# swift-nav/albatross

Measured on AMD Instinct MI355X. Metric: GP fits/sec (Gram+Chol+solve) at N=16384 fp64, higher is better.
Workload: dtype f64

## Files before the change

albatross_amd/csrc/api.hip:

```cpp
#include <algorithm>
#include <atomic>
#include <cmath>
#include <cstring>
#include <chrono>
#include <cstdio>
#include <new>
#include <thread>

#include "api_internal.h"
#include <deque>
#include <mutex>
#include <tuple>
#include <unordered_map>
#include "trace.h"
#include "pub.h"

namespace agp {

void DeviceFeatures::release() {
  for (void *&p : owned) {
    if (p) (void)hipFree(p);
    p = nullptr;
  }
  v = FeatView{};
// ... 146 lines not shown
  auto number = [](const char *name, long long dflt) {
    const char *e = getenv(name);
    return e && e[0] ? atoll(e) : dflt;
  };
  t.panel_fused = flag("AGP_PANEL_FUSED", true);
  t.step_below = number("AGP_STEP_BELOW", 4608);
  t.gram_sop = flag("AGP_GRAM_SOP", true);
  t.backsub_coop = flag("AGP_BACKSUB_COOP", true);
  t.backsub_coop_max = number("AGP_BACKSUB_COOP_MAX", BACKSUB_COOP_MAX_N);
  t.mixed_bf16 = flag("AGP_MIXED_BF16", true);
  t.mixed_f16 = flag("AGP_MIXED_F16", true);
  set_f16x2_kernel((int)number("AGP_F16X2_LDS_PAD", 8192), (int)number("AGP_F16X2_TERMS", 4), (int)number("AGP_F16X2_CHUNK", 32));
  t.mixed_nbo = number("AGP_MIXED_NBO", 512);
  t.fp64_nbo = number("AGP_FP64_NBO", 0);
  if (t.fp64_nbo <= 512 || t.fp64_nbo % 128 != 0) t.fp64_nbo = 0;
  set_bf16x3_kernel((int)number("AGP_BF16X3_KERNEL", 2), (int)number("AGP_BF16X3_LDS_PAD", 8192));
  t.sparse_pivoted = flag("AGP_SPARSE_PIVOTED", false);
  t.predict_chunk = number("AGP_PREDICT_CHUNK", 0);
  t.shard_block = number("AGP_SHARD_BLOCK", 0);
  t.shard_force_comm = flag("AGP_SHARD_FORCE_COMM", false);
  t.shard_host_pacing = flag("AGP_SHARD_HOST_PACING", false);
  if (const char *e = getenv("AGP_SHARD_MASK_GFLOP")) t.shard_mask_gflop = atof(e);
  t.merge_above = number("AGP_MERGE_ABOVE", 8704);
  return t;
}

int agp_context_create(int device_id, agp_context **out) {
  if (!out) return AGP_ERR_INVALID_ARGUMENT;
  *out = nullptr;
  int n = 0;
  if (hipGetDeviceCount(&n) != hipSuccess || n <= 0) return AGP_ERR_NO_DEVICE;
  if (device_id < 0 || device_id >= n) return AGP_ERR_INVALID_ARGUMENT;
  agp_context_impl *ctx = new (std::nothrow) agp_context_impl();
  if (!ctx) return AGP_ERR_INVALID_ARGUMENT;
  ctx->device = device_id;
  ctx->tune = read_tuning();
  agp::g_gram_sop = ctx->tune.gram_sop;
  AGP_HIP_CHECK(ctx, hipSetDevice(device_id));
  {
    int lo = 0, hi = 0;
    AGP_HIP_CHECK(ctx, hipDeviceGetStreamPriorityRange(&lo, &hi));
    AGP_HIP_CHECK(ctx, hipStreamCreateWithPriority(&ctx->stream, hipStreamNonBlocking, hi));
    AGP_HIP_CHECK(ctx, hipStreamCreateWithPriority(&ctx->stream2, hipStreamNonBlocking, lo));
    AGP_HIP_CHECK(ctx, hipStreamCreateWithPriority(&ctx->stream3, hipStreamNonBlocking, lo));
    AGP_HIP_CHECK(ctx, hipEventCreateWithFlags(&ctx->ev_inv, hipEventDisableTiming));
    AGP_HIP_CHECK(ctx, hipEventCreateWithFlags(&ctx->ev_c, hipEventDisableTiming));
// ... 33 lines not shown
  ctx->helpers.clear();
  for (auto &sl : ctx->ext.slots)
    if (sl.dev) (void)hipFree(sl.dev);
  for (auto e : ctx->gemm_events) (void)hipEventDestroy(e);
  for (auto e : ctx->stage_ev)
    if (e) (void)hipEventDestroy(e);
  if (ctx->partial_ws) (void)hipFree(ctx->partial_ws);
  if (ctx->ws_A) (void)agp::dev_release(ctx->ws_A);
  if (ctx->pool_A) (void)agp::dev_release(ctx->pool_A);
  if (ctx->pool_K) (void)agp::dev_release(ctx->pool_K);
  if (ctx->ws_refine) (void)hipFree(ctx->ws_refine);
  if (ctx->p32) (void)hipFree(ctx->p32);
  if (ctx->f16_scales) (void)hipFree(ctx->f16_scales);
  if (ctx->pool_L32) (void)hipFree(ctx->pool_L32);
  if (ctx->pool_aux) (void)agp::dev_release(ctx->pool_aux);
  if (ctx->pool_shard) (void)agp::dev_release(ctx->pool_shard);
  if (ctx->pool_sparse) (void)agp::dev_release(ctx->pool_sparse);
  if (ctx->pool_batch) (void)agp::dev_release(ctx->pool_batch);
  if (ctx->ws_aux) (void)hipFree(ctx->ws_aux);
  if (ctx->d_zpub) (void)hipFree(ctx->d_zpub);
  if (ctx->d_dpub) (void)hipFree(ctx->d_dpub);
  if (ctx->shard_flags) (void)hipFree(ctx->shard_flags);
  if (ctx->d_headcnt) (void)hipFree(ctx->d_headcnt);
  if (ctx->h_stage) (void)hipHostFree(ctx->h_stage);
  if (ctx->d_flags) (void)hipFree(ctx->d_flags);
  if (ctx->h_flags) (void)hipHostFree(ctx->h_flags);
  if (ctx->ev_a) (void)hipEventDestroy(ctx->ev_a);
  if (ctx->ev_b) (void)hipEventDestroy(ctx->ev_b);
  if (ctx->stream) (void)hipStreamDestroy(ctx->stream);
  if (ctx->stream2) (void)hipStreamDestroy(ctx->stream2);
  if (ctx->stream3) (void)hipStreamDestroy(ctx->stream3);
  if (ctx->ev_inv) (void)hipEventDestroy(ctx->ev_inv);
  if (ctx->stream_masked) (void)hipStreamDestroy(ctx->stream_masked);
  if (ctx->stream_comm) (void)hipStreamDestroy(ctx->stream_comm);
  if (ctx->ev_c) (void)hipEventDestroy(ctx->ev_c);
  delete ctx;
  agp::dev_cache_trim();
}

int agp_context_synchronize(agp_context *ctx) {
  if (!ctx) return AGP_ERR_INVALID_ARGUMENT;
  AGP_HIP_CHECK(ctx, hipSetDevice(ctx->device));
  AGP_HIP_CHECK(ctx, hipDeviceSynchronize());
  return AGP_OK;
}

// ... 1652 lines not shown
```

albatross_amd/csrc/chol.hip:

```cpp
#include <cstdlib>
#include "common.h"
#include "mfma_f64.h"
#include "gemm_tiles.h"
#include "trsm_kernel.h"
#include "pub.h"

namespace agp {
void launch_set_identity_batched(hipStream_t s, double *B, long long ld, long long stride, long long m, long long count);

__device__ __forceinline__ double readlane_f64(double v, int lane) {
  const long long b = __double_as_longlong(v);
  const int lo = __builtin_amdgcn_readlane((int)(b & 0xffffffffll), lane);
  const int hi = __builtin_amdgcn_readlane((int)(b >> 32), lane);
  return __longlong_as_double(((long long)hi << 32) | (unsigned int)lo);
}

__device__ __forceinline__ double rsqrt_nr(double x) {
  double y = __builtin_amdgcn_rsq(x);
  const double h = 0.5 * x;
  y = y * (1.5 - h * y * y);
  y = y * (1.5 - h * y * y);
  return y;
}

struct PotrfArgs {
  double *A;
  long long lda;
  long long k0;
  int nbk;
  double *img;
  double *y;
// ... 803 lines not shown
  const long long cnt_img = (b1 - b0) * (long long)IMG_DOUBLES, cnt_z = k_end - k_begin;
  if (ctx->d_dpub && ctx->dpub_cap >= b1) {
    prep->fill(ctx->d_rowcnt + 2 * b0, 0ull, 2 * (b1 - b0));
    prep->sentinel(ctx->d_dpub + b0 * (long long)IMG_DOUBLES, cnt_img);
  }
  prep->sentinel(invd + b0 * (long long)IMG_DOUBLES, cnt_img);
  prep->sentinel(ctx->d_zpub + k_begin, cnt_z);
  if (want_step && k_begin == 0 && ctx->d_headcnt && ctx->tune.merge_above > 0 && k_end > ctx->tune.merge_above && !prep->full()) {
    prep->fill(ctx->d_headcnt, 0ull, agp_context::HEADCNT_WORDS);
    ctx->headcnt_ready = true;
  }
  ctx->zpub_ready_n = k_end;
  ctx->img_ready = invd;
  return true;
}

void panel_fused_prepare(agp_context *ctx, hipStream_t s, double *invd, long long k_begin, long long k_end, bool want_step) {
  PrepArgs prep;
  if (panel_fused_plan(ctx, invd, k_begin, k_end, want_step, &prep)) launch_prep(s, prep);
}

static void panel_phase(agp_context *ctx, hipStream_t s, double *A, long long n, long long lda, double *invd,
                        double *y, long long K0, long long kend, FactorTimers *timers, bool step_mode = false,
                        long long mark_after = -1, hipEvent_t mark_event = nullptr) {
  if (kend != n) step_mode = false;
  const bool inner_left = !step_mode && (n - K0) > INNER_LEFT_ABOVE;
  const bool fused = ctx->tune.panel_fused && ctx->d_zpub && ctx->zpub_ready_n >= kend && ctx->img_ready == invd &&
                     ((n - K0) <= FUSED_BELOW || step_mode);
  for (long long k = K0; k < kend; k += NB) {
    const int nbk = (int)((n - k < NB) ? n - k : NB);
    if (mark_event && k == mark_after + NB) (void)hipEventRecord(mark_event, s);
    if (inner_left && k > K0) {
      const double *P = A + K0 * lda + k;
      timed_gemm(s, timers, A + k * lda + k, lda, P, P, n - k, nbk, k - K0, false);
    }
    const long long below = n - (k + nbk);
    if (fused) {
      PotrfArgs pa;
      pa.A = A; pa.lda = lda; pa.k0 = k; pa.nbk = nbk;
      pa.img = invd + (k / NB) * (long long)IMG_DOUBLES;
      pa.y = y ? y + k : nullptr;
      pa.flags = ctx->d_flags; pa.scalars = ctx->d_scalars;
      pa.zpub = y ? ctx->d_zpub + k : nullptr;
      pa.below = below > 0 ? below : 0;
      if (step_mode && k > K0) {
        pa.dpub = ctx->d_dpub + (k / NB) * (long long)IMG_DOUBLES;
        unsigned grid = (unsigned)(1 + UPD_BLOCKS + (pa.below + 63) / 64);
        if (pa.below > 0) {
          const long long nt = (pa.below + 63) / 64;
          pa.trail_first = grid;
// ... 32 lines not shown
      ++ctx->sched.panels_split;
      if (below <= 0) continue;
      TrsmArgs t;
      t.img = invd + (k / NB) * (long long)IMG_DOUBLES;
      t.nbk = nbk;
      t.Y = A + k * lda + (k + nbk);
      t.stride_m = lda; t.stride_n = 1;
      t.ncols = below;
      t.z = y ? y + k : nullptr;
      t.yrest = y ? y + k + nbk : nullptr;
      t.batch_img = t.batch_Y = 0; t.n_total = 0;
      const unsigned grid = (unsigned)((below + 63) / 64);
      if (y) hipLaunchKernelGGL((trsm_micro_kernel<false, true>), dim3(grid), dim3(256), 0, s, t);
      else hipLaunchKernelGGL((trsm_micro_kernel<false, false>), dim3(grid), dim3(256), 0, s, t);
    }
    const long long width = kend - (k + nbk);
    if (width > 0 && !inner_left && !(step_mode && fused)) {
      const double *P = A + k * lda + (k + nbk);
      timed_gemm(s, timers, A + (k + nbk) * lda + (k + nbk), lda, P, P, below, width, nbk, false);
    }
  }
}

__global__ __launch_bounds__(64) void head_gate_kernel(const unsigned long long *done, unsigned long long expect, int *flags) {
  if (threadIdx.x == 0) {
    const unsigned long long t0 = __builtin_amdgcn_s_memrealtime();
    for (int spin = 1; __hip_atomic_load(done, __ATOMIC_RELAXED, __HIP_MEMORY_SCOPE_AGENT) < expect; ++spin) {
      if ((spin & 63) == 0 && poll_expired(t0, flags)) break;
      __builtin_amdgcn_s_sleep(16);
    }
    __atomic_thread_fence(__ATOMIC_ACQUIRE);
  }
}

void launch_head_gate(hipStream_t s, const unsigned long long *done, unsigned long long expect, int *flags) {
  hipLaunchKernelGGL(head_gate_kernel, dim3(1), dim3(64), 0, s, done, expect, flags);
}

static bool host_wait_event(hipEvent_t ev) {
  for (;;) {
    const hipError_t e = hipEventQuery(ev);
    if (e == hipSuccess) return true;
    if (e != hipErrorNotReady) { (void)hipGetLastError(); return false; }
    for (int i = 0; i < 32; ++i) __builtin_ia32_pause();
  }
}
// ... 48 lines not shown
  hipStream_t sa = ctx->stream, sb = ctx->stream2;
  hipStream_t sb_prev = sb;
  bool have_u2 = false, p32_flip = false;
  agp_context::ScheduleRecord &rec = ctx->sched;
  rec.reset_factor(n);
  long long K0 = 0, step_index = 0;
  const long long nbo_fixed = ctx->nbo_override;
  int variant = ctx->update_variant;
  const double *rs16 = nullptr, *irs16 = nullptr;
  if (variant == 5) {
    if (ctx->f16_scales && ctx->f16_scales_n >= n) {
      launch_f16x2_row_scales(sa, A, lda, n, ctx->f16_scales, ctx->f16_scales + ctx->f16_scales_n);
      rs16 = ctx->f16_scales;
      irs16 = ctx->f16_scales + ctx->f16_scales_n;
    } else {
      variant = 4;
    }
  }
  const long long nbo_wide = (variant == 4 || variant == 5) ? ctx->nbo_wide : ctx->tune.fp64_nbo;
  long long kend = K0 + pick_nbo(n, nbo_fixed, nbo_wide);
  if (kend > n) kend = n;
  if (!(ctx->prep_external && ctx->img_ready == invd && ctx->zpub_ready_n >= n)) panel_fused_prepare(ctx, sa, invd, 0, n, true);
  ctx->prep_external = false;
  auto step_ok = [&](long long remaining) { return nbo_fixed == 0 && step_fits(ctx, remaining) && step_ready(ctx, invd, n); };
  const bool step_all = step_ok(n);
  if (step_all) kend = n;
  const bool early_inv = step_all && ctx->bs_W && ctx->bs_done == 0 && ctx->ev_inv && ctx->stream2 && ctx->bs_BW > 0 &&
                         n % ctx->bs_BW == 0 && n / ctx->bs_BW >= 2;
  rec.add_step(kend, step_all ? rec.STEP : 0u);
  panel_phase(ctx, sa, A, n, lda, invd, y, K0, kend, timers, step_all, early_inv ? (n / ctx->bs_BW - 1) * ctx->bs_BW - NB : -1,
              early_inv ? ctx->ev_c : nullptr);
  if (early_inv) {
    const long long BW = ctx->bs_BW, done = n / BW - 1;
    if (host_wait_event(ctx->ev_c)) {
      hipStream_t si = ctx->stream2;
      launch_set_identity_batched(si, ctx->bs_W, BW, BW * BW, BW, done);
      forward_solve_mat_batched(si, A, BW * (lda + 1), BW, lda, invd, (BW / NB) * (long long)IMG_DOUBLES, ctx->bs_W, BW * BW, BW, BW,
                                true, done);
      (void)hipEventRecord(ctx->ev_inv, si);
      ctx->bs_done = done;
      rec.inv_bits |= rec.INV_EARLY;
    }
  }
  while (kend < n) {
    long long next_end = kend + pick_nbo(n - kend, nbo_fixed, nbo_wide);
    if (next_end > n) next_end = n;
    const long long K = kend - K0;
    const bool step = step_ok(n - kend);
    const bool single = !step && nbo_fixed == 0 && n - kend <= SINGLE_BELOW;
    if (step || single) next_end = n;
    if (ctx->bs_W && ctx->bs_done == 0 && next_end == n && ctx->ev_inv && ctx->stream2) {
      const long long BW = ctx->bs_BW, done = kend / BW;
      if (done > 0) {
        hipStream_t si = ctx->stream2;
        (void)hipEventRecord(ctx->ev_c, sa);
        (void)hipStreamWaitEvent(si, ctx->ev_c, 0);
        if (have_u2) (void)hipStreamWaitEvent(si, ctx->ev_b, 0);
        launch_set_identity_batched(si, ctx->bs_W, BW, BW * BW, BW, done);
        forward_solve_mat_batched(si, A, BW * (lda + 1), BW, lda, invd, (BW / NB) * (long long)IMG_DOUBLES, ctx->bs_W, BW * BW, BW, BW,
                                  true, done);
        (void)hipEventRecord(ctx->ev_inv, si);
        ctx->bs_done = done;
        rec.inv_bits |= rec.INV_LAST_STEP;
      }
    }
    const double *P = A + K0 * lda + kend;
    const float *P32 = nullptr;
    long long ld32 = 0;
    const unsigned short *P16 = nullptr;
    if (variant == 3 && ctx->p32 && (n - kend) >= U1_F32_ABOVE) {
      ld32 = (n - kend + 7) / 8 * 8;
      if (ld32 % 512 == 0) ld32 += 8;
      if (sizeof(float) * (size_t)ld32 * (size_t)K * 2 <= ctx->p32_bytes) {
        float *dst = ctx->p32 + (size_t)(p32_flip ? 1 : 0) * (ctx->p32_bytes / sizeof(float) / 2);
        p32_flip = !p32_flip;
        launch_convert_panel_f32(sa, P, lda, n - kend, K, dst, ld32);
        P32 = dst;
      }
    } else if (variant == 4 && ctx->p32 && (n - kend) >= U1_F32_ABOVE && K % 32 == 0 && 2 * bf16x3_bytes(n - kend, K) <= ctx->p32_bytes) {
      unsigned short *dst = reinterpret_cast<unsigned short *>(ctx->p32) + (size_t)(p32_flip ? 1 : 0) * (ctx->p32_bytes / sizeof(unsigned short) / 2);
      p32_flip = !p32_flip;
      launch_convert_panel_bf16x3(sa, P, lda, n - kend, K, dst);
      P16 = dst;
// ... 6 lines not shown
    (void)hipEventRecord(ctx->ev_a, sa);
    const bool merged = variant <= 0 && nbo_fixed == 0 && !step && next_end < n && ctx->headcnt_ready && ctx->tune.merge_above > 0 &&
                        (n - kend) > ctx->tune.merge_above && step_index < agp_context::HEADCNT_WORDS && (next_end - kend) % NB == 0;
    if (merged) {
      sb = (ctx->stream_masked && (n - kend) <= MASK_BELOW) ? ctx->stream_masked : ctx->stream2;
      if (sb != sb_prev && have_u2) (void)hipStreamWaitEvent(sb, ctx->ev_b, 0);
      sb_prev = sb;
      (void)hipStreamWaitEvent(sb, ctx->ev_a, 0);
      BulkTiming bt;
      const bool timed = timers && timers->ev && timers->used + 2 <= timers->n_ev;
      if (timed) { bt.e0 = timers->ev[timers->used]; bt.e1 = timers->ev[timers->used + 1]; }
      long long head_tiles = 0;
      unsigned long long *cnt = ctx->d_headcnt + step_index;
      launch_trailing_update_merged(sb, A + kend * lda + kend, lda, P, lda, n - kend, K, (int)((next_end - kend) / NB), cnt, &head_tiles,
                                    timed ? &bt : nullptr);
      if (timed && bt.flops > 0.) {
        timers->flops[timers->used / 2] = bt.flops;
        timers->used += 2;
      }
      (void)hipEventRecord(ctx->ev_b, sb);
      have_u2 = true;
      launch_head_gate(sa, cnt, (unsigned long long)head_tiles, ctx->d_flags);
      rec.add_step(next_end, rec.MERGED | (sb == ctx->stream_masked ? rec.MASKED : 0u));
      panel_phase(ctx, sa, A, n, lda, invd, y, kend, next_end, timers, false);
      K0 = kend;
      kend = next_end;
      ++step_index;
      continue;
    }
    ++step_index;
    if (have_u2) (void)hipStreamWaitEvent(sa, ctx->ev_b, 0);
    if (P16 && variant == 5) {
      launch_update_f16x2(sa, A + kend * lda + kend, lda, P16, n - kend, 0, 0, irs16 + kend, n - kend, next_end - kend, K);
    } else if (P16) {
      launch_update_bf16x3(sa, A + kend * lda + kend, lda, P16, n - kend, 0, 0, n - kend, next_end - kend, K);
    } else if ((variant == 3 || variant == 4 || variant == 5) && (n - kend) >= U1_F32_ABOVE) {
      launch_update_f32(sa, A + kend * lda + kend, lda, P, P, lda, n - kend, next_end - kend, K, P32, P32, ld32);
    } else if (step && n - kend > 1536) {
      timed_gemm(sa, timers, A + kend * lda + kend, lda, P, P, n - kend, n - kend, K, true, variant >= 4 ? 3 : variant);
    } else {
      timed_gemm(sa, timers, A + kend * lda + kend, lda, P, P, n - kend, next_end - kend, K, false);
    }
    sb = (ctx->stream_masked && (n - kend) <= MASK_BELOW) ? ctx->stream_masked : ctx->stream2;
    if (sb != sb_prev && have_u2) (void)hipStreamWaitEvent(sb, ctx->ev_b, 0);
    sb_prev = sb;
    const bool throttle = next_end < n && (n - kend) <= THROTTLE_BELOW;
    rec.add_step(next_end, (step ? rec.STEP : 0u) | (throttle ? rec.THROTTLED : 0u) | (single ? rec.SINGLE : 0u) |
                               (next_end < n && sb == ctx->stream_masked ? rec.MASKED : 0u));
    if (throttle) panel_phase(ctx, sa, A, n, lda, invd, y, kend, next_end, timers, step);
    if (next_end < n) {
      if (throttle) {
        if (!host_wait_event(ctx->ev_a)) (void)hipStreamWaitEvent(sb, ctx->ev_a, 0);
      } else {
        (void)hipStreamWaitEvent(sb, ctx->ev_a, 0);
      }
      const double *Q = A + K0 * lda + next_end;
      if (P16) {
        const long long M2 = n - next_end;
        const int ntr = (int)((M2 + 127) / 128);
        const long long tiles = (long long)ntr * (ntr + 1) / 2;
        long long olen = 0;
        const int *order = tiles >= 1024 ? bulk_tile_order(ntr, tiles, &olen) : nullptr;
        if (variant == 5)
          launch_update_f16x2(sb, A + next_end * lda + next_end, lda, P16, n - kend, next_end - kend, next_end - kend, irs16 + kend, M2, M2, K,
                              order, olen);
        else
          launch_update_bf16x3(sb, A + next_end * lda + next_end, lda, P16, n - kend, next_end - kend, next_end - kend, M2, M2, K, order, olen);
      } else
      timed_gemm(sb, timers, A + next_end * lda + next_end, lda, Q, Q, n - next_end, n - next_end, K, true, variant >= 4 ? 3 : variant,
                 P32 ? P32 + (next_end - kend) : nullptr, ld32);
      (void)hipEventRecord(ctx->ev_b, sb);
      have_u2 = true;
    } else {
      have_u2 = false;
    }
    const long long bw = ctx->bs_BW;
    const bool tail_inv = !throttle && step && next_end == n && ctx->bs_W && bw > 0 && ctx->ev_inv && ctx->stream2 && n % bw == 0 &&
                          ctx->bs_done > 0 && ctx->bs_done == kend / bw && n / bw - 1 > ctx->bs_done && (n / bw - 1) * bw - NB >= kend;
    if (!throttle) panel_phase(ctx, sa, A, n, lda, invd, y, kend, next_end, timers, step, tail_inv ? (n / bw - 1) * bw - NB : -1,
                               tail_inv ? ctx->ev_c : nullptr);
    if (tail_inv) {
      const long long first = ctx->bs_done, last = n / bw - 1, cnt = last - first;
      if (host_wait_event(ctx->ev_c)) {
        hipStream_t si = ctx->stream2;
        launch_set_identity_batched(si, ctx->bs_W + first * bw * bw, bw, bw * bw, bw, cnt);
        forward_solve_mat_batched(si, A + first * bw * (lda + 1), bw * (lda + 1), bw, lda, invd + first * (bw / NB) * (long long)IMG_DOUBLES,
                                  (bw / NB) * (long long)IMG_DOUBLES, ctx->bs_W + first * bw * bw, bw * bw, bw, bw, true, cnt);
        (void)hipEventRecord(ctx->ev_inv, si);
        ctx->bs_done = last;
        rec.inv_bits |= rec.INV_TAIL;
      }
    }
    K0 = kend;
    kend = next_end;
  }
  ctx->img_ready = nullptr;
  ctx->headcnt_ready = false;
}

bool batched_fused_fits(agp_context *ctx, long long n, long long count) {
  if (!ctx->tune.panel_fused || n <= NB) return false;
  const long long per_problem = 1 + (n - NB + 63) / 64;
  return count * per_problem <= step_slots(ctx);
}

void factor_lower_batched(hipStream_t s, double *A, long long stride_A, long long n, long long lda, double *invd,
                          long long stride_invd, double *y, long long stride_y, long long count, int *flags,
                          double *logsum, long long stride_flags, double *zpub, long long stride_zpub) {
  if (count <= 0 || n <= 0) return;
  const bool fused = zpub != nullptr && y != nullptr;
  for (long long K0 = 0; K0 < n; K0 += NBO) {
    const long long kend = (K0 + NBO < n) ? K0 + NBO : n;
    for (long long k = K0; k < kend; k += NB) {
      const int nbk = (int)((n - k < NB) ? n - k : NB);
      if (k > K0) {
        const double *P = A + K0 * lda + k;
        launch_gemm_nt_sub_batched(s, A + k * lda + k, lda, stride_A, P, lda, false, stride_A, P, lda, false, stride_A, n - k, nbk,
// ... 102 lines not shown
```

albatross_amd/csrc/common.h:

```cpp
#pragma once
#include <hip/hip_runtime.h>
#include <cstdint>
#include <cstdio>
#include <string>
#include <utility>
#include <vector>

#include "../../include/albatross_amd.h"
#include "cov_eval.h"

#define AGP_CHAIN_PRIO 3

namespace agp {

constexpr int NB = 128;
constexpr int NBO = 512;
constexpr int MB = 16;
constexpr int NMB = NB / MB;

struct FeatView {
  const double *coords;
  const long long *ids;
  const double *scales;
  long long n;
// ... 68 lines not shown
  double *d_zpub = nullptr;
  long long zpub_cap = 0, zpub_ready_n = 0;
  double *d_dpub = nullptr;
  long long dpub_cap = 0;
  int cus = 256;
  long long step_slots = 0;
  struct Tuning {
    bool panel_fused = true;
    long long step_below = 4608;
    bool gram_sop = true;
    long long fp64_nbo = 0;
    long long mixed_nbo = 512;
    bool mixed_f16 = true;
    bool mixed_bf16 = true;
    long long backsub_coop_max = 2047;
    bool backsub_coop = true;
    bool sparse_pivoted = false;
    long long predict_chunk = 0;
    long long shard_block = 0;
    bool shard_force_comm = false;
    bool shard_host_pacing = false;
    double shard_mask_gflop = 40.;
    long long merge_above = 8704;
  } tune;
  unsigned long long *d_rowcnt = nullptr;
  void *h_stage = nullptr;
  size_t h_stage_bytes = 0;
  static constexpr long long HEADCNT_WORDS = 256;
  unsigned long long *d_headcnt = nullptr;
  bool headcnt_ready = false;
  struct ScheduleRecord {
    static constexpr unsigned MERGED = 1, STEP = 2, THROTTLED = 4, MASKED = 8, SINGLE = 16;
    enum Backsub { BS_NONE = 0, BS_COOP_DIRECT = 1, BS_COOP_FLAGS = 2, BS_WIDE = 3, BS_CHAIN = 4 };
    static constexpr unsigned INV_EARLY = 1, INV_LAST_STEP = 2, INV_TAIL = 4;
    long long n = 0;
    long long steps = 0, steps_dropped = 0;
    long long kend[HEADCNT_WORDS] = {};
    unsigned bits[HEADCNT_WORDS] = {};
    long long panels_step = 0, panels_fused = 0, panels_split = 0;
    int backsub = BS_NONE;
    long long bs_done = 0;
    unsigned inv_bits = 0;
    int handover_timeout = 0;
    long long demotions = 0;
    void reset_factor(long long n_) {
      n = n_;
      steps = steps_dropped = 0;
      panels_step = panels_fused = panels_split = 0;
      inv_bits = 0;
      handover_timeout = 0;
    }
    void add_step(long long end, unsigned b) {
      if (steps < HEADCNT_WORDS) { kend[steps] = end; bits[steps] = b; ++steps; }
      else ++steps_dropped;
    }
  } sched;
  double *bs_W = nullptr;
  long long bs_BW = 0, bs_done = 0;
  hipEvent_t ev_inv = nullptr;
  const double *img_ready = nullptr;
  bool prep_external = false;
  hipStream_t stream_comm = nullptr;
  unsigned long long *shard_flags = nullptr;
  unsigned long long shard_seq[16] = {};
  unsigned long long shard_probe_seq = 0;
  int shard_host_pacing = -1;
  bool shard_probe_ok = false;
};

struct agp_fit_slab {
  double *base = nullptr;
  size_t bytes = 0;
  int refs = 0;
};

struct agp_fit {
  agp_context *ctx = nullptr;
  agp_fit_slab *slab = nullptr;
  size_t A_bytes = 0;
  int device = 0;
  int64_t n = 0;
// ... 91 lines not shown
                        double *B, long long m, long long ldb);
constexpr long long WIDE_BW = 512;
bool forward_solve_wide_ok(long long n, long long ncols);
void invert_wide_blocks(hipStream_t s, const double *A, long long n, long long lda, const double *invd, long long BW, double *W);
void forward_solve_wide(hipStream_t s, const double *A, long long n, long long lda, const double *Winv, const double *B,
                        long long ldb, double *X, long long ldx, long long ncols);

void launch_coldot(hipStream_t s, const double *A, long long lda, const double *B, long long ldb,
                   long long n, long long m, double *out, double scale, const double *base);
void launch_gemm_tn_sub(hipStream_t s, const double *V, long long ldv, const double *W, long long ldw,
                        long long n, long long m, double *C, long long ldc);
void launch_gemv_t(hipStream_t s, const double *A, long long lda, long long n, long long m,
                   const double *x, double *y);
void launch_dot(hipStream_t s, const double *a, const double *b, long long n, double *out);

}

namespace agp {
void launch_gemm_nt_sub(hipStream_t s, double *C, long long ldc, const double *A, long long lda,
                        bool a_kmajor, const double *B, long long ldb, bool b_kmajor, long long M,
                        long long N, long long K, bool tri);
void launch_gemm_nt_ext(hipStream_t s, double *C, long long ldc, const double *Cin, long long ldcin, const double *A, long long lda,
                        const double *B, long long ldb, long long M, long long N, long long K);
void launch_gemm_nt_sub_stair(hipStream_t s, double *C, long long ldc, const double *A, long long lda, const double *B,
                              long long ldb, long long M, long long N, long long K, int world, int rank, long long lb0,
                              long long block, long long c0);
struct BulkTiming {
  hipEvent_t e0 = nullptr, e1 = nullptr;
  double flops = 0.;
};
void launch_trailing_update_as(int variant, hipStream_t s, double *C, long long ldc, const double *P,
                               const double *Q, long long ldp, long long M, long long K,
                               BulkTiming *timing = nullptr, const float *P32 = nullptr, const float *Q32 = nullptr,
                               long long ld32 = 0);
void launch_trailing_update(hipStream_t s, double *C, long long ldc, const double *P, const double *Q,
                            long long ldp, long long M, long long K, BulkTiming *timing = nullptr);
void read_bulk_probe(unsigned long long *out);
void read_bf16_probe(unsigned long long *out);
void read_potrf_probe(unsigned long long *out);
void launch_head_gate(hipStream_t s, const unsigned long long *done, unsigned long long expect, int *flags);
void launch_trailing_update_merged(hipStream_t s, double *C, long long ldc, const double *P, long long ldp, long long M, long long K,
                                   int head_cols, unsigned long long *head_done, long long *head_tiles, BulkTiming *timing = nullptr);
void launch_update_f32(hipStream_t s, double *C, long long ldc, const double *P, const double *Q, long long ldp, long long M,
                       long long N, long long K, const float *P32 = nullptr, const float *Q32 = nullptr, long long ld32 = 0);
size_t bf16x3_bytes(long long rows, long long K);
void launch_convert_panel_bf16x3(hipStream_t s, const double *P, long long ldp, long long rows, long long K, unsigned short *planes);
// ... 16 lines not shown
```

albatross_amd/csrc/debug_api.hip:

```cpp
#include <algorithm>
#include <cstdio>
#include "common.h"
#include "api_internal.h"
#include "mfma_f64.h"
#include "shard_internal.h"
#include "pub.h"
#include "trsm_kernel.h"
#include <cstdlib>
#include <cstring>
#include <new>

#define AGP_DEBUG_API __attribute__((visibility("default")))

namespace agp {

__global__ void mfma_tile_kernel(const double *A, const double *B, double *D) {
  const int l = threadIdx.x;
  v4d acc = v4zero();
  acc = mfma16(A[(l & 15) * 4 + (l >> 4)], B[(l >> 4) * 16 + (l & 15)], acc);
  for (int r = 0; r < 4; ++r) D[((l >> 4) + 4 * r) * 16 + (l & 15)] = acc[r];
}

template <int NACC>
__global__ __launch_bounds__(256) void mfma_clock_kernel(unsigned long long *out, int iters, double a0, double b0) {
// ... 1033 lines not shown
  factor_lower(ctx, dA, n, lda, dI, dy, nullptr);
  AGP_HIP_CHECK(ctx, hipStreamSynchronize(ctx->stream));
  AGP_HIP_CHECK(ctx, hipGetLastError());
  AGP_HIP_CHECK(ctx, hipMemcpy(A, dA, ab, hipMemcpyDeviceToHost));
  if (y) AGP_HIP_CHECK(ctx, hipMemcpy(y, dy, sizeof(double) * (size_t)n, hipMemcpyDeviceToHost));
  int flags[4];
  double scal[4];
  AGP_HIP_CHECK(ctx, hipMemcpy(flags, ctx->d_flags, sizeof(flags), hipMemcpyDeviceToHost));
  AGP_HIP_CHECK(ctx, hipMemcpy(scal, ctx->d_scalars, sizeof(scal), hipMemcpyDeviceToHost));
  if (log_det) *log_det = 2. * scal[0];
  if (bad_pivot) *bad_pivot = flags[1] ? flags[1] - 1 : -1;
  (void)hipFree(dA); (void)hipFree(dI);
  if (dy) (void)hipFree(dy);
  ctx->sched.backsub = agp_context::ScheduleRecord::BS_NONE;
  ctx->sched.bs_done = 0;
  ctx->sched.handover_timeout = flags[2];
  return AGP_OK;
}

constexpr int64_t SCHED_HEADER = 20;
AGP_DEBUG_API int agp_debug_schedule(agp_context *ctx, int64_t *out, int64_t cap) {
  if (!ctx || !out || cap < 0) return AGP_ERR_INVALID_ARGUMENT;
  const agp_context::ScheduleRecord &r = ctx->sched;
  int64_t w[SCHED_HEADER + 2 * agp_context::HEADCNT_WORDS] = {};
  w[0] = r.n; w[1] = r.steps; w[2] = r.steps_dropped;
  w[3] = r.panels_step; w[4] = r.panels_fused; w[5] = r.panels_split;
  w[6] = r.backsub; w[7] = r.bs_done; w[8] = r.inv_bits; w[9] = r.handover_timeout; w[10] = r.demotions;
  w[11] = ctx->step_slots; w[12] = ctx->cus; w[13] = ctx->stream_masked ? 1 : 0;
  w[14] = ctx->tune.step_below; w[15] = ctx->tune.panel_fused ? 1 : 0; w[16] = ctx->tune.merge_above;
  w[17] = ctx->tune.backsub_coop ? 1 : 0; w[18] = ctx->tune.fp64_nbo;
  for (long long i = 0; i < r.steps; ++i) {
    w[SCHED_HEADER + 2 * i] = r.kend[i];
    w[SCHED_HEADER + 2 * i + 1] = r.bits[i];
  }
  const int64_t total = SCHED_HEADER + 2 * agp_context::HEADCNT_WORDS;
  for (int64_t i = 0; i < cap && i < total; ++i) out[i] = w[i];
  return AGP_OK;
}

}

namespace agp {
__global__ __launch_bounds__(256) void mfma_peak_kernel(double *sink, int iters, double a0, double b0) {
  v4d acc[8];
#pragma unroll
  for (int i = 0; i < 8; ++i) acc[i] = v4zero();
  double a = a0 + threadIdx.x * 1e-9, b = b0 - threadIdx.x * 1e-9;
  for (int it = 0; it < iters; ++it) {
#pragma unroll
    for (int i = 0; i < 8; ++i) acc[i] = mfma16(a, b, acc[i]);
  }
  double s = 0.;
#pragma unroll
  for (int i = 0; i < 8; ++i) s += acc[i][0] + acc[i][1] + acc[i][2] + acc[i][3];
  if (s == 123.456) sink[0] = s;
}

static int mfma_f64_peak(hipStream_t s, int iters, double *tflops) {
// ... 75 lines not shown
```

albatross_amd/csrc/gemm.hip:

```cpp
#include <cmath>
#include <cstdlib>
#include <algorithm>
#include <map>
#include <mutex>
#include <tuple>
#include <vector>
#include "common.h"
#include "mfma_f64.h"
#include "gemm_tiles.h"

namespace agp {




__device__ __forceinline__ bool tile_of_block(const GemmArgs &g, int &bi, int &bj) {
  if (g.stair) {
    const long long id = blockIdx.x;
    bi = (int)(id % g.ntr);
    bj = (int)(id / g.ntr);
    const long long lb = g.st_lb0 + bi / g.st_tpb;
    const long long gi = lb * g.st_world + ((lb & 1) ? g.st_world - 1 - g.st_rank : g.st_rank);
    return bj <= gi * g.st_tpb - g.st_c0t + (bi % g.st_tpb);
  }
// ... 12 lines not shown
template <bool A_KMAJOR, bool B_KMAJOR>
__device__ __forceinline__ void gemm_nt_sub_body(const GemmArgs &g, double *lds) {
  int bi, bj;
  if (!tile_of_block(g, bi, bj)) return;
  if (tile_takes_cpf(g, bi, bj)) gemm_nt_sub_tile_cpf<A_KMAJOR, B_KMAJOR>(g, bi, bj, lds);
  else gemm_nt_sub_tile<A_KMAJOR, B_KMAJOR>(g, bi, bj, lds);
}

template <bool A_KMAJOR, bool B_KMAJOR>
__global__ __launch_bounds__(GEMM_THREADS, 2) void gemm_nt_sub_kernel(GemmArgs g) {
  __builtin_amdgcn_s_setprio(AGP_CHAIN_PRIO);
  g.C += (long long)blockIdx.y * g.batch_C;
  g.A += (long long)blockIdx.y * g.batch_A;
  g.B += (long long)blockIdx.y * g.batch_B;
  __shared__ double lds[2 * 2 * GK * GLD];
  gemm_nt_sub_body<A_KMAJOR, B_KMAJOR>(g, lds);
}

__global__ __launch_bounds__(GEMM_THREADS, 2) void gemm_nt_ext_kernel(GemmArgs g) {
  __shared__ double lds[2 * 2 * GK * GLD];
  const int bi = (int)(blockIdx.x % g.ntr), bj = (int)(blockIdx.x / g.ntr);
  if (tile_takes_cpf(g, bi, bj)) gemm_nt_sub_tile_cpf<false, true, true>(g, bi, bj, lds);
  else gemm_nt_sub_tile<false, true, true>(g, bi, bj, lds);
}

#ifdef AGP_BULK_STAMPS
__device__ unsigned long long g_bulk_probe[4];
void read_bulk_probe(unsigned long long *out) { (void)hipMemcpyFromSymbol(out, HIP_SYMBOL(g_bulk_probe), sizeof(unsigned long long) * 4); }
#else
void read_bulk_probe(unsigned long long *out) { for (int i = 0; i < 4; ++i) out[i] = 0; }
#endif

__global__ __launch_bounds__(GEMM_THREADS, 2) void trailing_update_kernel(GemmArgs g) {
  __shared__ double lds[2 * 2 * GK * GLD];
#ifdef AGP_BULK_STAMPS
  const unsigned long long stamp_c0 = __builtin_amdgcn_s_memtime(), stamp_r0 = __builtin_amdgcn_s_memrealtime();
#endif
  long long wg = blockIdx.x;
  const bool head = wg < g.head_count;
  int bi, bj = 0;
  if (head) {
    const int nth = g.ntr + g.head_cols;
    long long id = wg;
    while (id >= nth - bj) {
      id -= nth - bj;
      ++bj;
// ... 408 lines not shown
  if ((long long)g.ntr * g.ntc / 2 < 4LL * slots) {
    g.ntr = (int)((M + ST - 1) / ST);
    g.ntc = (int)((N + ST - 1) / ST);
    g.st_tpb = (int)(block / ST);
    g.st_c0t = c0 / ST;
    hipLaunchKernelGGL(gemm64_nt_sub_kernel, dim3((unsigned)((long long)g.ntr * g.ntc)), dim3(GEMM_THREADS), 0, s, g);
    return;
  }
  hipLaunchKernelGGL((gemm_nt_sub_kernel<false, false>), dim3((unsigned)((long long)g.ntr * g.ntc)), dim3(GEMM_THREADS), 0, s, g);
}

void launch_gemm_nt_ext(hipStream_t s, double *C, long long ldc, const double *Cin, long long ldcin, const double *A, long long lda,
                        const double *B, long long ldb, long long M, long long N, long long K) {
  if (M <= 0 || N <= 0 || K <= 0) return;
  GemmArgs g;
  g.C = C; g.ldc = ldc; g.A = A; g.lda = lda; g.B = B; g.ldb = ldb;
  g.M = M; g.N = N; g.K = K; g.tri = 0;
  g.ntr = (int)((M + GT - 1) / GT);
  g.ntc = (int)((N + GT - 1) / GT);
  g.Cin = Cin; g.ldcin = ldcin; g.assign = Cin ? 0 : 1;
  hipLaunchKernelGGL(gemm_nt_ext_kernel, dim3((unsigned)((long long)g.ntr * g.ntc)), dim3(GEMM_THREADS), 0, s, g);
}

void launch_gemm_nt_sub(hipStream_t s, double *C, long long ldc, const double *A, long long lda,
                        bool a_kmajor, const double *B, long long ldb, bool b_kmajor, long long M,
                        long long N, long long K, bool tri) {
  launch_gemm_nt_sub_batched(s, C, ldc, 0, A, lda, a_kmajor, 0, B, ldb, b_kmajor, 0, M, N, K, tri, 1);
}

static double lower_entries(long long M, int ntr, long long count) {
  double e = 0.;
  for (int bj = 0; bj < ntr && count > 0; ++bj) {
    const long long w = (M - (long long)bj * GT < GT) ? M - (long long)bj * GT : GT;
    for (int bi = bj; bi < ntr && count > 0; ++bi, --count) {
      const long long h = (M - (long long)bi * GT < GT) ? M - (long long)bi * GT : GT;
      e += (bi == bj) ? 0.5 * (double)w * (double)(w + 1) : (double)h * (double)w;
    }
  }
  return e;
}

struct XcdOrder { int *dev = nullptr; long long len = 0; };
static XcdOrder xcd_order(int ntr, long long full) {
  static std::mutex mu;
  static std::map<std::tuple<int, int, long long>, XcdOrder> cache;
  int device = 0;
// ... 184 lines not shown
```

Measured before the change: 34.68.

## Factor wide 512-column panels via diagonal-block inverse and GEMM instead of TRSM

For large trailing sizes, outer panels are fixed at 512 columns. Each panel is factored only over its diagonal block, the inverse of that diagonal block is formed by a forward solve, and the rows below are then updated as a triangular GEMM against the inverse (in-place, column blocks processed in reverse). The RHS update becomes a tall matvec. The inverse can also be stored into the back-substitution workspace so later backsub inverses are not recomputed. The aim is to replace the latency-bound per-panel TRSM with MFMA GEMM work. In exchange it disables the fused and step panel modes for these sizes and adds explicit-inverse numerical error.

Result: slower. 32.92 (-5.1%).

```diff
diff --git a/albatross_amd/csrc/api.hip b/albatross_amd/csrc/api.hip
--- a/albatross_amd/csrc/api.hip
+++ b/albatross_amd/csrc/api.hip
@@ -192,6 +192,9 @@
   t.shard_host_pacing = flag("AGP_SHARD_HOST_PACING", false);
   if (const char *e = getenv("AGP_SHARD_MASK_GFLOP")) t.shard_mask_gflop = atof(e);
   t.merge_above = number("AGP_MERGE_ABOVE", 8704);
+  t.wide_panel_above = number("AGP_WIDE_PANEL_ABOVE", 8704);
+  if (t.wide_panel_above < 0) t.wide_panel_above = 0;
+  t.wide_panel_reuse = flag("AGP_WIDE_PANEL_REUSE", true);
   return t;
 }
 
@@ -271,6 +274,7 @@
   if (ctx->d_dpub) (void)hipFree(ctx->d_dpub);
   if (ctx->shard_flags) (void)hipFree(ctx->shard_flags);
   if (ctx->d_headcnt) (void)hipFree(ctx->d_headcnt);
+  if (ctx->d_wide_W) (void)hipFree(ctx->d_wide_W);
   if (ctx->h_stage) (void)hipHostFree(ctx->h_stage);
   if (ctx->d_flags) (void)hipFree(ctx->d_flags);
   if (ctx->h_flags) (void)hipHostFree(ctx->h_flags);
diff --git a/albatross_amd/csrc/chol.hip b/albatross_amd/csrc/chol.hip
--- a/albatross_amd/csrc/chol.hip
+++ b/albatross_amd/csrc/chol.hip
@@ -7,6 +7,8 @@
 
 namespace agp {
 void launch_set_identity_batched(hipStream_t s, double *B, long long ld, long long stride, long long m, long long count);
+void launch_tall_matvec(hipStream_t s, const double *W, long long ld, long long rows, long long ncols, const double *x, double alpha,
+                        double beta, const double *base, double *out);
 
 __device__ __forceinline__ double readlane_f64(double v, int lane) {
   const long long b = __double_as_longlong(v);
@@ -856,10 +858,10 @@
 
 static void panel_phase(agp_context *ctx, hipStream_t s, double *A, long long n, long long lda, double *invd,
                         double *y, long long K0, long long kend, FactorTimers *timers, bool step_mode = false,
-                        long long mark_after = -1, hipEvent_t mark_event = nullptr) {
+                        long long mark_after = -1, hipEvent_t mark_event = nullptr, bool allow_fused = true) {
   if (kend != n) step_mode = false;
   const bool inner_left = !step_mode && (n - K0) > INNER_LEFT_ABOVE;
-  const bool fused = ctx->tune.panel_fused && ctx->d_zpub && ctx->zpub_ready_n >= kend && ctx->img_ready == invd &&
+  const bool fused = allow_fused && ctx->tune.panel_fused && ctx->d_zpub && ctx->zpub_ready_n >= kend && ctx->img_ready == invd &&
                      ((n - K0) <= FUSED_BELOW || step_mode);
   for (long long k = K0; k < kend; k += NB) {
     const int nbk = (int)((n - k < NB) ? n - k : NB);
@@ -938,6 +940,19 @@
   }
 }
 
+static void wide_panel_phase(agp_context *ctx, hipStream_t s, double *A, long long n, long long lda, double *invd, double *y,
+                             long long K0, long long kend, FactorTimers *timers, double *W) {
+  const long long bw = kend - K0, below = n - kend;
+  panel_phase(ctx, s, A, kend, lda, invd, y, K0, kend, timers, false, -1, nullptr, false);
+  if (below <= 0) return;
+  launch_set_identity_batched(s, W, bw, bw * bw, bw, 1);
+  forward_solve_mat_batched(s, A + K0 * (lda + 1), 0, bw, lda, invd + (K0 / NB) * (long long)IMG_DOUBLES, 0, W, 0, bw, bw,
+                            true, 1);
+  double *X = A + K0 * lda + kend;
+  launch_panel_times_inverse(s, X, lda, below, W, bw, bw);
+  if (y) launch_tall_matvec(s, X, lda, below, bw, y + K0, -1.0, 1.0, y + kend, y + kend);
+}
+
 __global__ __launch_bounds__(64) void head_gate_kernel(const unsigned long long *done, unsigned long long expect, int *flags) {
   if (threadIdx.x == 0) {
     const unsigned long long t0 = __builtin_amdgcn_s_memrealtime();
@@ -1032,14 +1047,43 @@
   if (kend > n) kend = n;
   if (!(ctx->prep_external && ctx->img_ready == invd && ctx->zpub_ready_n >= n)) panel_fused_prepare(ctx, sa, invd, 0, n, true);
   ctx->prep_external = false;
-  auto step_ok = [&](long long remaining) { return nbo_fixed == 0 && step_fits(ctx, remaining) && step_ready(ctx, invd, n); };
+  const long long wide_above = (variant <= 0 && nbo_fixed == 0) ? ctx->tune.wide_panel_above : 0;
+  auto wide_rows = [&](long long remaining) { return wide_above > 0 && remaining > wide_above && remaining > 512; };
+  if (wide_rows(n) && !ctx->d_wide_W && hipMalloc(&ctx->d_wide_W, sizeof(double) * 512 * 512) != hipSuccess) {
+    (void)hipGetLastError();
+    ctx->d_wide_W = nullptr;
+  }
+  const bool wide_on = wide_rows(n) && ctx->d_wide_W;
+  auto wide_ok = [&](long long k0, long long k1) { return wide_on && k1 - k0 == 512 && wide_rows(n - k0); };
+  auto nbo_of = [&](long long remaining) {
+    const long long w = pick_nbo(remaining, nbo_fixed, nbo_wide);
+    return (w < 512 && wide_on && wide_rows(remaining)) ? 512 : w;
+  };
+  long long wide_inv = 0;
+  auto run_panel_phase = [&](long long k0, long long k1, bool step_mode, long long mark_after, hipEvent_t mark_event) {
+    if (!wide_ok(k0, k1)) {
+      panel_phase(ctx, sa, A, n, lda, invd, y, k0, k1, timers, step_mode, mark_after, mark_event);
+      return;
+    }
+    double *W = ctx->d_wide_W;
+    if (ctx->tune.wide_panel_reuse && ctx->bs_W && ctx->bs_done == 0 && ctx->bs_BW == 512 && n % 512 == 0 && k0 / 512 == wide_inv &&
+        n - k1 > 0 && ctx->ev_inv) {
+      W = ctx->bs_W + wide_inv * 512 * 512;
+      ++wide_inv;
+    }
+    wide_panel_phase(ctx, sa, A, n, lda, invd, y, k0, k1, timers, W);
+    if (rec.steps > 0 && rec.steps <= agp_context::HEADCNT_WORDS) rec.bits_ext[rec.steps - 1] |= rec.WIDE_PANEL;
+  };
+  if (wide_on) kend = K0 + nbo_of(n);
+  auto step_ok = [&](long long remaining) {
+    return nbo_fixed == 0 && !(wide_on && wide_rows(remaining)) && step_fits(ctx, remaining) && step_ready(ctx, invd, n);
+  };
   const bool step_all = step_ok(n);
   if (step_all) kend = n;
   const bool early_inv = step_all && ctx->bs_W && ctx->bs_done == 0 && ctx->ev_inv && ctx->stream2 && ctx->bs_BW > 0 &&
                          n % ctx->bs_BW == 0 && n / ctx->bs_BW >= 2;
   rec.add_step(kend, step_all ? rec.STEP : 0u);
-  panel_phase(ctx, sa, A, n, lda, invd, y, K0, kend, timers, step_all, early_inv ? (n / ctx->bs_BW - 1) * ctx->bs_BW - NB : -1,
-              early_inv ? ctx->ev_c : nullptr);
+  run_panel_phase(K0, kend, step_all, early_inv ? (n / ctx->bs_BW - 1) * ctx->bs_BW - NB : -1, early_inv ? ctx->ev_c : nullptr);
   if (early_inv) {
     const long long BW = ctx->bs_BW, done = n / BW - 1;
     if (host_wait_event(ctx->ev_c)) {
@@ -1053,22 +1097,25 @@
     }
   }
   while (kend < n) {
-    long long next_end = kend + pick_nbo(n - kend, nbo_fixed, nbo_wide);
+    long long next_end = kend + nbo_of(n - kend);
     if (next_end > n) next_end = n;
     const long long K = kend - K0;
     const bool step = step_ok(n - kend);
-    const bool single = !step && nbo_fixed == 0 && n - kend <= SINGLE_BELOW;
+    const bool single = !step && nbo_fixed == 0 && n - kend <= SINGLE_BELOW && !(wide_on && wide_rows(n - kend));
     if (step || single) next_end = n;
     if (ctx->bs_W && ctx->bs_done == 0 && next_end == n && ctx->ev_inv && ctx->stream2) {
-      const long long BW = ctx->bs_BW, done = kend / BW;
+      const long long BW = ctx->bs_BW, done = kend / BW, first = wide_inv < done ? wide_inv : done;
       if (done > 0) {
         hipStream_t si = ctx->stream2;
         (void)hipEventRecord(ctx->ev_c, sa);
         (void)hipStreamWaitEvent(si, ctx->ev_c, 0);
         if (have_u2) (void)hipStreamWaitEvent(si, ctx->ev_b, 0);
-        launch_set_identity_batched(si, ctx->bs_W, BW, BW * BW, BW, done);
-        forward_solve_mat_batched(si, A, BW * (lda + 1), BW, lda, invd, (BW / NB) * (long long)IMG_DOUBLES, ctx->bs_W, BW * BW, BW, BW,
-                                  true, done);
+        if (done > first) {
+          launch_set_identity_batched(si, ctx->bs_W + first * BW * BW, BW, BW * BW, BW, done - first);
+          forward_solve_mat_batched(si, A + first * BW * (lda + 1), BW * (lda + 1), BW, lda, invd + first * (BW / NB) * (long long)IMG_DOUBLES,
+                                    (BW / NB) * (long long)IMG_DOUBLES, ctx->bs_W + first * BW * BW, BW * BW, BW, BW, true,
+                                    done - first);
+        }
         (void)hipEventRecord(ctx->ev_inv, si);
         ctx->bs_done = done;
         rec.inv_bits |= rec.INV_LAST_STEP;
@@ -1121,7 +1168,7 @@
       have_u2 = true;
       launch_head_gate(sa, cnt, (unsigned long long)head_tiles, ctx->d_flags);
       rec.add_step(next_end, rec.MERGED | (sb == ctx->stream_masked ? rec.MASKED : 0u));
-      panel_phase(ctx, sa, A, n, lda, invd, y, kend, next_end, timers, false);
+      run_panel_phase(kend, next_end, false, -1, nullptr);
       K0 = kend;
       kend = next_end;
       ++step_index;
@@ -1146,7 +1193,7 @@
     const bool throttle = next_end < n && (n - kend) <= THROTTLE_BELOW;
     rec.add_step(next_end, (step ? rec.STEP : 0u) | (throttle ? rec.THROTTLED : 0u) | (single ? rec.SINGLE : 0u) |
                                (next_end < n && sb == ctx->stream_masked ? rec.MASKED : 0u));
-    if (throttle) panel_phase(ctx, sa, A, n, lda, invd, y, kend, next_end, timers, step);
+    if (throttle) run_panel_phase(kend, next_end, step, -1, nullptr);
     if (next_end < n) {
       if (throttle) {
         if (!host_wait_event(ctx->ev_a)) (void)hipStreamWaitEvent(sb, ctx->ev_a, 0);
@@ -1176,8 +1223,7 @@
     const long long bw = ctx->bs_BW;
     const bool tail_inv = !throttle && step && next_end == n && ctx->bs_W && bw > 0 && ctx->ev_inv && ctx->stream2 && n % bw == 0 &&
                           ctx->bs_done > 0 && ctx->bs_done == kend / bw && n / bw - 1 > ctx->bs_done && (n / bw - 1) * bw - NB >= kend;
-    if (!throttle) panel_phase(ctx, sa, A, n, lda, invd, y, kend, next_end, timers, step, tail_inv ? (n / bw - 1) * bw - NB : -1,
-                               tail_inv ? ctx->ev_c : nullptr);
+    if (!throttle) run_panel_phase(kend, next_end, step, tail_inv ? (n / bw - 1) * bw - NB : -1, tail_inv ? ctx->ev_c : nullptr);
     if (tail_inv) {
       const long long first = ctx->bs_done, last = n / bw - 1, cnt = last - first;
       if (host_wait_event(ctx->ev_c)) {
@@ -1192,6 +1238,10 @@
     }
     K0 = kend;
     kend = next_end;
+  }
+  if (wide_inv > 0 && ctx->bs_done == 0 && ctx->ev_inv) {
+    (void)hipEventRecord(ctx->ev_inv, sa);
+    ctx->bs_done = wide_inv;
   }
   ctx->img_ready = nullptr;
   ctx->headcnt_ready = false;
diff --git a/albatross_amd/csrc/common.h b/albatross_amd/csrc/common.h
--- a/albatross_amd/csrc/common.h
+++ b/albatross_amd/csrc/common.h
@@ -114,6 +114,8 @@
     bool shard_host_pacing = false;
     double shard_mask_gflop = 40.;
     long long merge_above = 8704;
+    long long wide_panel_above = 8704;
+    bool wide_panel_reuse = true;
   } tune;
   unsigned long long *d_rowcnt = nullptr;
   void *h_stage = nullptr;
@@ -123,12 +125,14 @@
   bool headcnt_ready = false;
   struct ScheduleRecord {
     static constexpr unsigned MERGED = 1, STEP = 2, THROTTLED = 4, MASKED = 8, SINGLE = 16;
+    static constexpr unsigned WIDE_PANEL = 32;
     enum Backsub { BS_NONE = 0, BS_COOP_DIRECT = 1, BS_COOP_FLAGS = 2, BS_WIDE = 3, BS_CHAIN = 4 };
     static constexpr unsigned INV_EARLY = 1, INV_LAST_STEP = 2, INV_TAIL = 4;
     long long n = 0;
     long long steps = 0, steps_dropped = 0;
     long long kend[HEADCNT_WORDS] = {};
     unsigned bits[HEADCNT_WORDS] = {};
+    unsigned bits_ext[HEADCNT_WORDS] = {};
     long long panels_step = 0, panels_fused = 0, panels_split = 0;
     int backsub = BS_NONE;
     long long bs_done = 0;
@@ -143,12 +147,13 @@
       handover_timeout = 0;
     }
     void add_step(long long end, unsigned b) {
-      if (steps < HEADCNT_WORDS) { kend[steps] = end; bits[steps] = b; ++steps; }
+      if (steps < HEADCNT_WORDS) { kend[steps] = end; bits[steps] = b; bits_ext[steps] = 0; ++steps; }
       else ++steps_dropped;
     }
   } sched;
   double *bs_W = nullptr;
   long long bs_BW = 0, bs_done = 0;
+  double *d_wide_W = nullptr;
   hipEvent_t ev_inv = nullptr;
   const double *img_ready = nullptr;
   bool prep_external = false;
@@ -286,6 +291,7 @@
                         long long N, long long K, bool tri);
 void launch_gemm_nt_ext(hipStream_t s, double *C, long long ldc, const double *Cin, long long ldcin, const double *A, long long lda,
                         const double *B, long long ldb, long long M, long long N, long long K);
+void launch_panel_times_inverse(hipStream_t s, double *X, long long ldx, long long M, const double *W, long long ldw, long long bw);
 void launch_gemm_nt_sub_stair(hipStream_t s, double *C, long long ldc, const double *A, long long lda, const double *B,
                               long long ldb, long long M, long long N, long long K, int world, int rank, long long lb0,
                               long long block, long long c0);
diff --git a/albatross_amd/csrc/debug_api.hip b/albatross_amd/csrc/debug_api.hip
--- a/albatross_amd/csrc/debug_api.hip
+++ b/albatross_amd/csrc/debug_api.hip
@@ -1079,7 +1079,8 @@
 AGP_DEBUG_API int agp_debug_schedule(agp_context *ctx, int64_t *out, int64_t cap) {
   if (!ctx || !out || cap < 0) return AGP_ERR_INVALID_ARGUMENT;
   const agp_context::ScheduleRecord &r = ctx->sched;
-  int64_t w[SCHED_HEADER + 2 * agp_context::HEADCNT_WORDS] = {};
+  constexpr int64_t EXT = SCHED_HEADER + 2 * agp_context::HEADCNT_WORDS;
+  int64_t w[EXT + 1 + agp_context::HEADCNT_WORDS] = {};
   w[0] = r.n; w[1] = r.steps; w[2] = r.steps_dropped;
   w[3] = r.panels_step; w[4] = r.panels_fused; w[5] = r.panels_split;
   w[6] = r.backsub; w[7] = r.bs_done; w[8] = r.inv_bits; w[9] = r.handover_timeout; w[10] = r.demotions;
@@ -1089,8 +1090,10 @@
   for (long long i = 0; i < r.steps; ++i) {
     w[SCHED_HEADER + 2 * i] = r.kend[i];
     w[SCHED_HEADER + 2 * i + 1] = r.bits[i];
-  }
-  const int64_t total = SCHED_HEADER + 2 * agp_context::HEADCNT_WORDS;
+    w[EXT + 1 + i] = r.bits_ext[i];
+  }
+  w[EXT] = ctx->tune.wide_panel_above;
+  const int64_t total = EXT + 1 + agp_context::HEADCNT_WORDS;
   for (int64_t i = 0; i < cap && i < total; ++i) out[i] = w[i];
   return AGP_OK;
 }
diff --git a/albatross_amd/csrc/gemm.hip b/albatross_amd/csrc/gemm.hip
--- a/albatross_amd/csrc/gemm.hip
+++ b/albatross_amd/csrc/gemm.hip
@@ -58,6 +58,14 @@
   const int bi = (int)(blockIdx.x % g.ntr), bj = (int)(blockIdx.x / g.ntr);
   if (tile_takes_cpf(g, bi, bj)) gemm_nt_sub_tile_cpf<false, true, true>(g, bi, bj, lds);
   else gemm_nt_sub_tile<false, true, true>(g, bi, bj, lds);
+}
+
+__global__ __launch_bounds__(GEMM_THREADS, 2) void panel_times_inverse_kernel(GemmArgs g) {
+  __builtin_amdgcn_s_setprio(AGP_CHAIN_PRIO);
+  __shared__ double lds[2 * 2 * GK * GLD];
+  const int bi = (int)blockIdx.x;
+  if (tile_takes_cpf(g, bi, 0)) gemm_nt_sub_tile_cpf<false, false, true>(g, bi, 0, lds);
+  else gemm_nt_sub_tile<false, false, true>(g, bi, 0, lds);
 }
 
 #ifdef AGP_BULK_STAMPS
@@ -512,6 +520,19 @@
   hipLaunchKernelGGL(gemm_nt_ext_kernel, dim3((unsigned)((long long)g.ntr * g.ntc)), dim3(GEMM_THREADS), 0, s, g);
 }
 
+void launch_panel_times_inverse(hipStream_t s, double *X, long long ldx, long long M, const double *W, long long ldw, long long bw) {
+  if (M <= 0 || bw <= 0 || bw % GT != 0) return;
+  for (long long bj = bw / GT - 1; bj >= 0; --bj) {
+    GemmArgs g;
+    g.C = X + bj * GT * ldx; g.ldc = ldx; g.A = X; g.lda = ldx; g.B = W + bj * GT; g.ldb = ldw;
+    g.M = M; g.N = GT; g.K = (bj + 1) * GT; g.tri = 0;
+    g.ntr = (int)((M + GT - 1) / GT);
+    g.ntc = 1;
+    g.assign = 1;
+    hipLaunchKernelGGL(panel_times_inverse_kernel, dim3((unsigned)g.ntr), dim3(GEMM_THREADS), 0, s, g);
+  }
+}
+
 void launch_gemm_nt_sub(hipStream_t s, double *C, long long ldc, const double *A, long long lda,
                         bool a_kmajor, const double *B, long long ldb, bool b_kmajor, long long M,
                         long long N, long long K, bool tri) {
```
